# dedis/kyber

Measured on AMD Instinct MI355X. Metric: scalar-muls/s + pairings/s per node; MSM sec at 2^20 points, higher is better.
Workload: dtype int32 limbs (radix 2^25.5), int64 accumulate; 1 GPU; Ed25519 batched fixed-base + var-base scalar-mul, 2^20 scalars per GPU (BASELINE.json configs[1]); elements_per_gpu=1048576

## Files before the change

kyber_amd/csrc/ed25519.hip:

```cpp
#ifndef KYB_TU_WAVES
#define KYB_TU_WAVES 2
#endif
#include "context.h"
#include "ed25519_dev.cuh"
#include "ed25519_launch.h"
#include "msm.cuh"
#include "ed25519_h2c.cuh"
#include <stdlib.h>
#include <string.h>

#include <algorithm>
#include <atomic>
#include <chrono>
#include <thread>
#include <vector>

namespace kyb {


template <int G = 2>
__global__ void ed25519_build_base_table_kernel(int32_t* __restrict__ tab, const uint32_t* __restrict__ point,
                                                uint32_t* __restrict__ ok, int rows = ED_TAB_POS * ED_TAB_ENT) {
    const int t = blockIdx.x * blockDim.x + threadIdx.x;
    if (t >= rows) return;
// ... 102 lines not shown
        ge_p3 h;
        ge_p3_0(h);
        ge_precomp t;
        ge_p1p1 r;
        EdCombDigits<1> digits(e);
#pragma unroll 1
        for (int i = 0; i < 64; i++) {
            select_precomp_uniform(t, tab, i, digits.next(i));
            ge_madd(r, h, t);
            ge_p1p1_to_p3(h, r);
        }
        if (proj) {
            store_proj(proj, idx, h);
            continue;
        }
        uint32_t w[8];
        ge_p3_towords(w, h);
        store_words8(out + idx * 8, w);
    }
}


template <bool GTAB, bool UNI = false>
__global__ __launch_bounds__(128, 3) void ed25519_mul_kernel(
    size_t n, const uint32_t* __restrict__ scalars, const uint32_t* __restrict__ points,
    size_t points_stride, uint32_t* __restrict__ out, uint8_t* __restrict__ status,
    uint32_t flags, int32_t* __restrict__ proj, int4* __restrict__ gtab) {
    const size_t idx = (size_t)blockIdx.x * blockDim.x + threadIdx.x;
    if (idx >= n) return;
    const bool full = !UNI && (flags & KYB_F_VARTIME) != 0;
    uint32_t pw[8], a[8];
    load_words8(pw, points + idx * points_stride);
    load_words8(a, scalars + idx * 8);
    ge_p3 A;
    const bool ok = ge_p3_fromwords(A, pw);
    int8_t e[65];
    recode16(e, a, full);
    ge_p3 h;
    const int vt_top = full ? wave_top_digit(a) : 63;
    if constexpr (GTAB) {
        TabGlobal tab{gtab + idx * 80};
        ge_scalarmult_w4<UNI, true>(h, e, A, full, tab, vt_top);
    } else {
        TabScratch tab;
        ge_scalarmult_w4<UNI, true>(h, e, A, full, tab, vt_top);
    }
    if (proj) {
        store_proj(proj, idx, h);
        if (status) status[idx] = ok ? KYB_ST_OK : KYB_ST_BAD_POINT;
        return;
    }
    uint32_t w[8];
    ge_p3_towords(w, h);
    if (!ok) {
#pragma unroll
        for (int i = 0; i < 8; i++) w[i] = 0;
    }
    store_words8(out + idx * 8, w);
    if (status) status[idx] = ok ? KYB_ST_OK : KYB_ST_BAD_POINT;
}

int ed25519_build_tables(DeviceCtx* ctx) {
    KYB_HIP_CHECK(hipMalloc(&ctx->ed_base_tab, ED_TAB_WORDS * sizeof(int32_t)));
    hipLaunchKernelGGL(ed25519_build_base_table_kernel<2>, dim3((ED_TAB_POS * ED_TAB_ENT + 63) / 64), dim3(64), 0,
                       nullptr, ctx->ed_base_tab, (const uint32_t*)nullptr, (uint32_t*)nullptr, ED_TAB_POS * ED_TAB_ENT);
    KYB_HIP_CHECK(hipGetLastError());
    const auto t0 = std::chrono::steady_clock::now();
    KYB_HIP_CHECK(hipMalloc(&ctx->ed_wide_tab, ED_WIDE_WORDS * sizeof(int32_t)));
    hipLaunchKernelGGL(ed25519_build_base_table_kernel<ED_COMB_G>, dim3((EdWide::ROWS + 63) / 64), dim3(64), 0, nullptr,
                       ctx->ed_wide_tab, (const uint32_t*)nullptr, (uint32_t*)nullptr, EdWide::ROWS);
    KYB_HIP_CHECK(hipGetLastError());
    KYB_HIP_CHECK(hipStreamSynchronize(nullptr));
    ctx->ed_wide_build_us = std::chrono::duration_cast<std::chrono::microseconds>(std::chrono::steady_clock::now() - t0).count();
    return KYB_OK;
}
void ed25519_free_tables(DeviceCtx* ctx) {
    if (ctx->ed_base_tab) hipFree(ctx->ed_base_tab);
// ... 588 lines not shown
```

kyber_amd/csrc/ed25519_dev.cuh:

```cuda
#pragma once
#include "ge25519.cuh"

#if !defined(__HIPCC__)
#include <type_traits>
struct int4 { int32_t x, y, z, w; };
struct uint4 { uint32_t x, y, z, w; };
inline int4 make_int4(int32_t x, int32_t y, int32_t z, int32_t w) { return int4{x, y, z, w}; }
inline uint4 make_uint4(uint32_t x, uint32_t y, uint32_t z, uint32_t w) { return uint4{x, y, z, w}; }
#define KYB_DEV_CONST static
#else
#define KYB_DEV_CONST __device__
#endif

namespace kyb {

constexpr int ED_TAB_POS = 33;
constexpr int ED_TAB_ENT = 136;
constexpr int ED_TAB_STRIDE = 32;
constexpr int ED_TAB_WORDS = ED_TAB_POS * ED_TAB_ENT * ED_TAB_STRIDE;

template <int G>
struct EdComb {
    static constexpr int POS = (65 + G - 1) / G;
    static constexpr int POS_CT = (64 + G - 1) / G;
// ... 43 lines not shown
        ge_p1p1_to_p3(acc, r);
    }
    fe zi, x, y, ypx, ymx, xy2d, z;
    fe_invert(zi, acc.Z);
    fe_mul(x, acc.X, zi);
    fe_mul(y, acc.Y, zi);
    fe_add(ypx, y, x);
    fe_sub(ymx, y, x);
    fe_mul(xy2d, x, y);
    fe_mul(xy2d, xy2d, fe_d2());
    fe_1(z);
    fe_mul(ypx, ypx, z);
    fe_mul(ymx, ymx, z);
#pragma unroll
    for (int l = 0; l < 10; l++) {
        o[l] = ypx.v[l];
        o[10 + l] = ymx.v[l];
        o[20 + l] = xy2d.v[l];
    }
    o[30] = o[31] = 0;
}

constexpr int ENC_CHUNK = 16;

KYB_DEV void store_proj(int32_t* __restrict__ proj, size_t idx, const ge_p3& h) {
    int32_t* o = proj + idx * 30;
#pragma unroll
    for (int l = 0; l < 10; l++) {
        o[l] = h.X.v[l];
        o[10 + l] = h.Y.v[l];
        o[20 + l] = h.Z.v[l];
    }
}
KYB_DEV void load_fe(fe& f, const int32_t* __restrict__ p) {
#pragma unroll
    for (int l = 0; l < 10; l++) f.v[l] = p[l];
}
struct EncPreScratch {
    fe pre[ENC_CHUNK];
    KYB_DEV void put(int j, const fe& f) { pre[j] = f; }
    KYB_DEV void get(fe& f, int j) const { f = pre[j]; }
};
template <int LANES>
struct EncPreLds {
    int32_t* col;
    static constexpr int WORDS = ENC_CHUNK * 10 * LANES;
    KYB_DEV void put(int j, const fe& f) {
#pragma unroll
        for (int l = 0; l < 10; l++) col[(j * 10 + l) * LANES] = f.v[l];
    }
    KYB_DEV void get(fe& f, int j) const {
#pragma unroll
        for (int l = 0; l < 10; l++) f.v[l] = col[(j * 10 + l) * LANES];
        KYB_FE_MAG_SET(f, 1.01);
    }
};
#if defined(__HIPCC__)
template <int GROUP = 1>
KYB_DEV size_t ed_encode_first() {
    return (size_t)blockIdx.x * blockDim.x * (ENC_CHUNK / GROUP) + threadIdx.x;
}
#endif
template <int GROUP = 1, class Pre, class Emit>
KYB_DEV void ed_encode_chunk(size_t n, const int32_t* __restrict__ proj, size_t first, size_t stride, Pre& pre, Emit emit) {
    static_assert(GROUP >= 1 && ENC_CHUNK % GROUP == 0, "whole records per lane");
    int cnt = 0;
// ... 69 lines not shown
    }
}

template <int G>
struct EdCombDigits {
    static_assert(G >= 1 && G <= 7, "a position's digits are read from one 32-bit word");
    static constexpr int PACKED = 63 / G;
    static constexpr int TAIL = EdComb<G>::POS - PACKED;
    uint32_t pk[8];
    int tail[TAIL];
    KYB_DEV explicit EdCombDigits(const int8_t e[65]) {
        ed_pack_digits(pk, e);
#pragma unroll
        for (int t = 0; t < TAIL; t++) {
            int d = 0;
#pragma unroll
            for (int i = G - 1; i >= 0; i--)
                if (G * (PACKED + t) + i <= 64) d = 16 * d + (int)e[G * (PACKED + t) + i];
            tail[t] = d;
        }
    }
    KYB_DEV int next(int k) {
        int d = (int)(pk[0] & ((1u << (4 * G)) - 1u)) - EdComb<G>::ENT;
#pragma unroll
        for (int j = 0; j < 7; j++) pk[j] = (pk[j] >> (4 * G)) | (pk[j + 1] << (32 - 4 * G));
        pk[7] >>= 4 * G;
#pragma unroll
        for (int t = 0; t < TAIL; t++)
            if (k == PACKED + t) d = tail[t];
        return d;
    }
};

struct TabScratch {
    ge_cached tab[8];
    KYB_DEV void put(int j, const ge_cached& c) { tab[j] = c; }
    KYB_DEV void get(ge_cached& c, int j) const { c = tab[j]; }
};
struct TabGlobal {
    int4* base;
    KYB_DEV void put(int j, const ge_cached& c) {
        int4* q = base + j * 10;
        const fe* f[4] = {&c.YpX, &c.YmX, &c.Z, &c.T2d};
        int32_t w[40];
#pragma unroll
        for (int k = 0; k < 4; k++)
#pragma unroll
            for (int l = 0; l < 10; l++) w[10 * k + l] = f[k]->v[l];
#pragma unroll
        for (int i = 0; i < 10; i++) q[i] = make_int4(w[4 * i], w[4 * i + 1], w[4 * i + 2], w[4 * i + 3]);
    }
    KYB_DEV void get(ge_cached& c, int j) const {
        const int4* q = base + j * 10;
        int32_t w[40];
#pragma unroll
        for (int i = 0; i < 10; i++) {
            const int4 x = q[i];
            w[4 * i] = x.x;
            w[4 * i + 1] = x.y;
            w[4 * i + 2] = x.z;
            w[4 * i + 3] = x.w;
        }
        fe* f[4] = {&c.YpX, &c.YmX, &c.Z, &c.T2d};
#pragma unroll
        for (int k = 0; k < 4; k++)
#pragma unroll
            for (int l = 0; l < 10; l++) f[k]->v[l] = w[10 * k + l];
    }
    KYB_DEV void get_signed(ge_cached& c, int b) const;
};
KYB_DEV_CONST __attribute__((aligned(16))) const int32_t ED_CACHED_IDENTITY[40] = {1, 0, 0, 0, 0, 0, 0, 0, 0, 0,
                                                                               1, 0, 0, 0, 0, 0, 0, 0, 0, 0,
                                                                               1};
KYB_DEV void TabGlobal::get_signed(ge_cached& c, int b) const {
    const bool neg = b < 0;
    const int babs = neg ? -b : b;
#if defined(__HIPCC__)
    typedef int32_t i32x2 __attribute__((ext_vector_type(2)));
    typedef int32_t i32x4 __attribute__((ext_vector_type(4)));
    using gint = const __attribute__((address_space(1))) int32_t;
    using gint2 = const __attribute__((address_space(1))) i32x2;
    using gint4 = const __attribute__((address_space(1))) i32x4;
#else
    struct i32x2 { int32_t x, y; };
    struct i32x4 { int32_t x, y, z, w; };
    using gint = const int32_t;
    using gint2 = const i32x2;
    using gint4 = const i32x4;
#endif
    gint* e = babs ? (gint*)(base + (babs - 1) * 10) : (gint*)ED_CACHED_IDENTITY;
    gint2* p = (gint2*)(e + (neg ? 10 : 0));
    gint2* m = (gint2*)(e + (neg ? 0 : 10));
    gint4* q = (gint4*)(e + 20);
#pragma unroll
    for (int i = 0; i < 5; i++) {
        const i32x2 x = p[i], y = m[i];
        c.YpX.v[2 * i] = x.x;
        c.YpX.v[2 * i + 1] = x.y;
        c.YmX.v[2 * i] = y.x;
        c.YmX.v[2 * i + 1] = y.y;
    }
    int32_t w[20];
#pragma unroll
    for (int i = 0; i < 5; i++) {
        const i32x4 x = q[i];
        w[4 * i] = x.x;
        w[4 * i + 1] = x.y;
        w[4 * i + 2] = x.z;
        w[4 * i + 3] = x.w;
    }
    const int32_t s = -(int32_t)neg;
#pragma unroll
    for (int l = 0; l < 10; l++) {
        c.Z.v[l] = w[l];
        c.T2d.v[l] = (w[10 + l] ^ s) - s;
    }
}
template <bool UNI = false, class Tab>
KYB_DEV void select_cached(ge_cached& c, const Tab& tab, int b) {
    const bool neg = b < 0;
    const int babs = neg ? -b : b;
    if constexpr (UNI) {
        ge_cached_0(c);
#pragma unroll 1
        for (int m = 1; m <= 8; m++) {
            ge_cached x;
            tab.get(x, m - 1);
            const int32_t keep = -(int32_t)(babs == m);
#pragma unroll
            for (int l = 0; l < 10; l++) {
                c.YpX.v[l] ^= (c.YpX.v[l] ^ x.YpX.v[l]) & keep;
                c.YmX.v[l] ^= (c.YmX.v[l] ^ x.YmX.v[l]) & keep;
                c.Z.v[l] ^= (c.Z.v[l] ^ x.Z.v[l]) & keep;
                c.T2d.v[l] ^= (c.T2d.v[l] ^ x.T2d.v[l]) & keep;
            }
        }
    } else if constexpr (std::is_same_v<Tab, TabGlobal>) {
        tab.get_signed(c, b);
        return;
    } else {
        tab.get(c, babs ? babs - 1 : 0);
        if (babs == 0) ge_cached_0(c);
    }
    ge_cached_cneg(c, neg);
}

KYB_DEV int wave_top_digit(const uint32_t a[8]) {
    int bits = 0;
#pragma unroll
    for (int i = 0; i < 8; i++)
        if (a[i]) bits = 32 * i + 32 - __builtin_clz(a[i]);
    int t = (bits + 3) >> 2;
    if (t > 64) t = 64;
#if defined(__HIP_DEVICE_COMPILE__)
#pragma unroll
    for (int off = 32; off >= 1; off >>= 1) {
        const int o = __shfl_xor(t, off, 64);
        t = o > t ? o : t;
    }
    t = __builtin_amdgcn_readfirstlane(t);
#endif
    return t;
}

template <bool AFFINE = false, class Tab>
KYB_DEV void ge_window_table(Tab& tab, const ge_p3& A) {
    ge_p1p1 t;
    ge_p3 u;
    ge_cached c;
    ge_p3_to_cached(c, A);
    tab.put(0, c);
    if constexpr (AFFINE) {
        const ge_precomp a{c.YpX, c.YmX, c.T2d};
        u = A;
#pragma unroll 1
        for (int i = 0; i < 7; i++) {
            ge_madd(t, u, a);
            ge_p1p1_to_p3(u, t);
            ge_p3_to_cached(c, u);
            tab.put(i + 1, c);
        }
    } else {
#pragma unroll 1
        for (int i = 0; i < 7; i++) {
            ge_add(t, A, c);
            ge_p1p1_to_p3(u, t);
            ge_p3_to_cached(c, u);
            tab.put(i + 1, c);
        }
    }
}

template <bool UNI = false, bool AFFINE = false, class Tab>
KYB_DEV void ge_scalarmult_w4(ge_p3& h, const int8_t e[65], const ge_p3& A, bool full, Tab& tab, int vt_top) {
    ge_p1p1 t;
    ge_p3 u;
    ge_p2 r;
    ge_cached c;
    ge_window_table<AFFINE>(tab, A);
    ge_p3_0(u);
    int top = 63;
    if (full) top = vt_top;
    select_cached<UNI>(c, tab, e[top]);
    ge_add(t, u, c);
    uint32_t pk[8];
    ed_pack_digits(pk, e);
    auto shl4 = [&pk]() {
#pragma unroll
        for (int j = 7; j > 0; j--) pk[j] = (pk[j] << 4) | (pk[j - 1] >> 28);
        pk[0] <<= 4;
    };
#pragma unroll 1
    for (int i = top; i < 64; i++) shl4();
#pragma unroll 1
    for (int i = top - 1; i >= 0; i--) {
        const int d = (int)(pk[7] >> 28) - 8;
        shl4();
        ge_p1p1_to_p2(r, t);
        ge_dbl(t, r.X, r.Y, r.Z);
        ge_p1p1_to_p2(r, t);
        ge_dbl(t, r.X, r.Y, r.Z);
        ge_p1p1_to_p2(r, t);
        ge_dbl(t, r.X, r.Y, r.Z);
        ge_p1p1_to_p2(r, t);
        ge_dbl(t, r.X, r.Y, r.Z);
#if defined(__HIP_DEVICE_COMPILE__)
        if (!UNI && full && __ballot(d != 0) == 0) continue;
#endif
        ge_p1p1_to_p3(u, t);
        select_cached<UNI>(c, tab, d);
        ge_add(t, u, c);
// ... 6 lines not shown
```

kyber_amd/csrc/fe25519.cuh:

```cuda
#pragma once
#include "hd.h"

namespace kyb {

struct fe {
    int32_t v[10];
#if defined(KYB_FE_AUDIT)
    double mag = 2.0;
#endif
};

#if defined(KYB_FE_AUDIT)
inline double& fe_audit_max() {
    static double m = 0;
    return m;
}
inline double& fe_audit_max19() {
    static double m = 0;
    return m;
}
inline void fe_audit_note(double pf, double pg, double scale) {
    const double x = pf * pg * scale;
    if (x > fe_audit_max()) fe_audit_max() = x;
    if (pg > fe_audit_max19()) fe_audit_max19() = pg;
}
#define KYB_FE_MAG_SET(h, x) ((h).mag = (x))
#define KYB_FE_MAG(f) ((f).mag)
#define KYB_FE_NOTE(pf, pg, scale) fe_audit_note(pf, pg, scale)
#else
#define KYB_FE_MAG_SET(h, x) ((void)0)
#define KYB_FE_MAG(f) 0.0
#define KYB_FE_NOTE(pf, pg, scale) ((void)0)
#endif

#if defined(__HIPCC__)
#define KYB_DEV __device__ __forceinline__
#else
#define KYB_DEV inline
// ... 157 lines not shown
}
KYB_DEV void fe_sq_sel(fe& h, const fe& f, bool dbl) {
    KYB_FE_NOTE(KYB_FE_MAG(f), KYB_FE_MAG(f), 2.0);
    fe g = f;
    int32_t f2[10], f19[10], f38[10];
#pragma unroll
    for (int i = 0; i < 10; i++) {
        f2[i] = 2 * g.v[i];
        f19[i] = 19 * g.v[i];
        f38[i] = (int32_t)(2u * (uint32_t)f19[i]);
    }
    int64_t t[10];
#pragma unroll
    for (int k = 0; k < 10; k++) {
        int64_t acc = 0;
#pragma unroll
        for (int i = 0; i < 10; i++) {
            const int j = (k - i + 10) % 10;
            if (i > j) continue;
            const bool wrap = (i + j) >= 10;
            const bool both_odd = (i & 1) && (j & 1);
            const int32_t a = i == j ? g.v[i] : f2[i];
            const int32_t b = wrap ? (both_odd ? f38[j] : f19[j]) : (both_odd ? f2[j] : g.v[j]);
            acc += (int64_t)a * (int64_t)b;
        }
        t[k] = (dbl ? (acc + acc) : acc) + fe_bias(k);
    }
    fe_carry_store(h, t);
    KYB_FE_MAG_SET(h, 1.01);
}
KYB_DEV void fe_sq(fe& h, const fe& f) { fe_sq_t<false>(h, f); }
KYB_DEV void fe_sq2(fe& h, const fe& f) { fe_sq_t<true>(h, f); }

KYB_DEV void fe_sqn(fe& h, const fe& f, int n) {
    fe_sq(h, f);
#pragma unroll 1
    for (int i = 1; i < n; i++) fe_sq(h, h);
}

KYB_DEV void fe_pow_2_250_1(fe& out, fe& z11, const fe& z) {
    fe z2, z9, t, a5, a10, a20, a50, a100;
    fe_sq(z2, z);
    fe_sqn(t, z2, 2);
    fe_mul(z9, t, z);
    fe_mul(z11, z9, z2);
    fe_sq(t, z11);
    fe_mul(a5, t, z9);
    fe_sqn(t, a5, 5);
    fe_mul(a10, t, a5);
    fe_sqn(t, a10, 10);
    fe_mul(a20, t, a10);
    fe_sqn(t, a20, 20);
    fe_mul(t, t, a20);
    fe_sqn(t, t, 10);
    fe_mul(a50, t, a10);
    fe_sqn(t, a50, 50);
    fe_mul(a100, t, a50);
    fe_sqn(t, a100, 100);
    fe_mul(t, t, a100);
    fe_sqn(t, t, 50);
    fe_mul(out, t, a50);
}
KYB_DEV void fe_invert(fe& out, const fe& z) {
    fe t, z11;
    fe_pow_2_250_1(t, z11, z);
    fe_sqn(t, t, 5);
    fe_mul(out, t, z11);
}
KYB_DEV void fe_pow22523(fe& out, const fe& z) {
    fe t, z11;
    fe_pow_2_250_1(t, z11, z);
    fe_sqn(t, t, 2);
    fe_mul(out, t, z);
}

KYB_DEV void fe_towords(uint32_t w[8], const fe& f) {
    int32_t h[10];
#pragma unroll
    for (int i = 0; i < 10; i++) h[i] = f.v[i];
    int32_t q = (19 * h[9] + (1 << 24)) >> 25;
#pragma unroll
    for (int i = 0; i < 10; i++) q = (h[i] + q) >> ((i & 1) ? 25 : 26);
    h[0] += 19 * q;
#pragma unroll
    for (int i = 0; i < 9; i++) {
        const int w_ = (i & 1) ? 25 : 26;
        int32_t c = h[i] >> w_;
        h[i + 1] += c;
        h[i] -= c << w_;
    }
    h[9] &= (1 << 25) - 1;
    uint32_t u[10];
#pragma unroll
    for (int i = 0; i < 10; i++) u[i] = (uint32_t)h[i];
    w[0] = u[0] | (u[1] << 26);
    w[1] = (u[1] >> 6) | (u[2] << 19);
    w[2] = (u[2] >> 13) | (u[3] << 13);
    w[3] = (u[3] >> 19) | (u[4] << 6);
    w[4] = u[5] | (u[6] << 25);
    w[5] = (u[6] >> 7) | (u[7] << 19);
    w[6] = (u[7] >> 13) | (u[8] << 12);
    w[7] = (u[8] >> 20) | (u[9] << 6);
}
KYB_DEV void fe_fromwords(fe& h, const uint32_t w[8]) {
    h.v[0] = (int32_t)(w[0] & 0x3ffffff);
    h.v[1] = (int32_t)(((w[0] >> 26) | (w[1] << 6)) & 0x1ffffff);
    h.v[2] = (int32_t)(((w[1] >> 19) | (w[2] << 13)) & 0x3ffffff);
    h.v[3] = (int32_t)(((w[2] >> 13) | (w[3] << 19)) & 0x1ffffff);
    h.v[4] = (int32_t)((w[3] >> 6) & 0x3ffffff);
    h.v[5] = (int32_t)(w[4] & 0x1ffffff);
    h.v[6] = (int32_t)(((w[4] >> 25) | (w[5] << 7)) & 0x3ffffff);
    h.v[7] = (int32_t)(((w[5] >> 19) | (w[6] << 13)) & 0x1ffffff);
    h.v[8] = (int32_t)(((w[6] >> 12) | (w[7] << 20)) & 0x3ffffff);
    h.v[9] = (int32_t)((w[7] >> 6) & 0x1ffffff);
    KYB_FE_MAG_SET(h, 2.0);
}
KYB_DEV bool fe_isnegative(const fe& f) {
    uint32_t w[8];
    fe_towords(w, f);
    return w[0] & 1;
}
KYB_DEV bool fe_isnonzero(const fe& f) {
// ... 10 lines not shown
```

kyber_amd/csrc/ge25519.cuh:

```cuda
#pragma once
#include "fe25519.cuh"

namespace kyb {

struct ge_p2 { fe X, Y, Z; };
struct ge_p3 { fe X, Y, Z, T; };
struct ge_p1p1 { fe X, Y, Z, T; };
struct ge_cached { fe YpX, YmX, Z, T2d; };
struct ge_precomp { fe ypx, ymx, xy2d; };

#include "ed25519_consts.inc"

KYB_DEV void ge_p3_0(ge_p3& h) {
    fe_0(h.X);
    fe_1(h.Y);
    fe_1(h.Z);
    fe_0(h.T);
}
KYB_DEV void ge_cached_0(ge_cached& c) {
    fe_1(c.YpX);
    fe_1(c.YmX);
    fe_1(c.Z);
    fe_0(c.T2d);
}
KYB_DEV void ge_p1p1_to_p2(ge_p2& r, const ge_p1p1& p) {
    fe_mul(r.X, p.X, p.T);
    fe_mul(r.Y, p.Y, p.Z);
    fe_mul(r.Z, p.Z, p.T);
}
KYB_DEV void ge_p1p1_to_p3(ge_p3& r, const ge_p1p1& p) {
    fe_mul(r.X, p.X, p.T);
    fe_mul(r.Y, p.Y, p.Z);
    fe_mul(r.Z, p.Z, p.T);
    fe_mul(r.T, p.X, p.Y);
}
KYB_DEV void ge_p3_to_cached(ge_cached& r, const ge_p3& p) {
    fe_add(r.YpX, p.Y, p.X);
    fe_sub(r.YmX, p.Y, p.X);
    r.Z = p.Z;
    fe_mul(r.T2d, p.T, fe_d2());
}
KYB_DEV void ge_dbl(ge_p1p1& r, const fe& X, const fe& Y, const fe& Z) {
    fe t0;
    fe_sq(r.X, X);
    fe_sq(r.Z, Y);
    fe_sq2(r.T, Z);
    fe_add(r.Y, X, Y);
    fe_sq(t0, r.Y);
    fe_add(r.Y, r.Z, r.X);
    fe_sub(r.Z, r.Z, r.X);
    fe_sub(r.X, t0, r.Y);
    fe_sub(r.T, r.T, r.Z);
}
KYB_DEV void ge_add(ge_p1p1& r, const ge_p3& p, const ge_cached& q) {
    fe t0;
    fe_add(r.X, p.Y, p.X);
    fe_sub(r.Y, p.Y, p.X);
    fe_mul(r.Z, r.X, q.YpX);
    fe_mul(r.Y, r.Y, q.YmX);
    fe_mul(r.T, q.T2d, p.T);
    fe_mul(r.X, p.Z, q.Z);
    fe_add(t0, r.X, r.X);
    fe_sub(r.X, r.Z, r.Y);
    fe_add(r.Y, r.Z, r.Y);
    fe_add(r.Z, t0, r.T);
    fe_sub(r.T, t0, r.T);
}
KYB_DEV void ge_madd(ge_p1p1& r, const ge_p3& p, const ge_precomp& q) {
    fe t0;
    fe_add(r.X, p.Y, p.X);
    fe_sub(r.Y, p.Y, p.X);
    fe_mul(r.Z, r.X, q.ypx);
    fe_mul(r.Y, r.Y, q.ymx);
    fe_mul(r.T, q.xy2d, p.T);
    fe_add(t0, p.Z, p.Z);
    fe_sub(r.X, r.Z, r.Y);
    fe_add(r.Y, r.Z, r.Y);
    fe_add(r.Z, t0, r.T);
    fe_sub(r.T, t0, r.T);
}
KYB_DEV void ge_cached_cneg(ge_cached& c, bool neg) {
    fe_cswap(c.YpX, c.YmX, neg);
    fe nt;
    fe_neg(nt, c.T2d);
    fe_cmov(c.T2d, nt, neg);
}
KYB_DEV void ge_precomp_cneg(ge_precomp& c, bool neg) {
    fe_cswap(c.ypx, c.ymx, neg);
    fe nt;
    fe_neg(nt, c.xy2d);
    fe_cmov(c.xy2d, nt, neg);
}

KYB_DEV void ge_encode_with_zinv(uint32_t w[8], const fe& X, const fe& Y, const fe& zinv) {
    fe x, y;
    fe_mul(x, X, zinv);
    fe_mul(y, Y, zinv);
    fe_towords(w, y);
    w[7] ^= (uint32_t)fe_isnegative(x) << 31;
}
KYB_DEV void ge_p3_towords(uint32_t w[8], const ge_p3& p) {
    fe zi;
    fe_invert(zi, p.Z);
    ge_encode_with_zinv(w, p.X, p.Y, zi);
}
KYB_DEV bool ge_p3_fromwords(ge_p3& p, const uint32_t w[8]) {
    fe u, v, v3, vxx, check;
    fe_fromwords(p.Y, w);
    fe_1(p.Z);
    fe_sq(u, p.Y);
    fe_mul(v, u, fe_d());
    fe_sub(u, u, p.Z);
    fe_add(v, v, p.Z);
    fe_sq(v3, v);
    fe_mul(v3, v3, v);
    fe_sq(p.X, v3);
    fe_mul(p.X, p.X, v);
    fe_mul(p.X, p.X, u);
    fe_pow22523(p.X, p.X);
    fe_mul(p.X, p.X, v3);
    fe_mul(p.X, p.X, u);
    fe_sq(vxx, p.X);
    fe_mul(vxx, vxx, v);
    fe_sub(check, vxx, u);
    bool ok = true;
    if (fe_isnonzero(check)) {
        fe_add(check, vxx, u);
        ok = !fe_isnonzero(check);
        fe xs;
        fe_mul(xs, p.X, fe_sqrtm1());
        p.X = xs;
    }
    const bool sign = (w[7] >> 31) != 0;
    fe nx;
    fe_neg(nx, p.X);
    fe_cmov(p.X, nx, fe_isnegative(p.X) != sign);
    fe_mul(p.T, p.X, p.Y);
    return ok;
}

KYB_DEV void recode16(int8_t e[65], const uint32_t a[8], bool full256) {
    int carry = 0;
#pragma unroll
    for (int i = 0; i < 64; i++) {
        int d = (int)((a[i >> 3] >> ((i & 7) * 4)) & 15) + carry;
        if (i < 63) {
            carry = (d + 8) >> 4;
            d -= carry << 4;
        }
        e[i] = (int8_t)d;
    }
    int top = e[63];
    int c2 = 0;
    if (full256) {
        c2 = (top + 8) >> 4;
        top -= c2 << 4;
    } else if (top > 8) {
        top = 0;
    }
    e[63] = (int8_t)top;
    e[64] = (int8_t)c2;
}

KYB_DEV bool ed_effective_scalar(uint32_t (&k)[8]) {
    uint32_t c = 0, t7 = 0;
#pragma unroll
    for (int j = 0; j < 8; j++) {
// ... 21 lines not shown
```

kyber_amd/csrc/gen_consts.py:

```python
#!/usr/bin/env python3
import os

HERE = os.path.dirname(os.path.abspath(__file__))


def limbs_25_5(x):
    out, off = [], 0
    for i in range(10):
        w = 25 if i & 1 else 26
        out.append((x >> off) & ((1 << w) - 1))
        off += w
    assert off == 255 and x >> 255 == 0
    return out


def ed25519():
    p = 2**255 - 19
    d = (-121665 * pow(121666, p - 2, p)) % p
    sqrtm1 = pow(2, (p - 1) // 4, p)
    by = 4 * pow(5, p - 2, p) % p
    u, v = (by * by - 1) % p, (d * by * by + 1) % p
    bx = (u * pow(v, 3, p) * pow(u * pow(v, 7, p) % p, (p - 5) // 8, p)) % p
    if (v * bx * bx - u) % p:
        bx = bx * sqrtm1 % p
    assert (v * bx * bx - u) % p == 0
    if bx & 1:
        bx = p - bx
    a = (-486664) % p
    c1 = pow(a, (p + 3) // 8, p)
    if c1 * c1 % p != a:
        c1 = c1 * sqrtm1 % p
    assert c1 * c1 % p == a
    if c1 & 1:
        c1 = p - c1
    c2 = pow(2, (p + 3) // 8, p)
    consts = dict(d=d, d2=2 * d % p, sqrtm1=sqrtm1, bx=bx, by=by, bt=bx * by % p, elligator_c1=c1, elligator_c2=c2)
    lines = ["// generated by gen_consts.py -- do not edit"]
    for name, val in consts.items():
        ls = ", ".join(str(v) for v in limbs_25_5(val))
        lines.append(f"KYB_DEV fe fe_{name}() {{ return fe{{{{{ls}}}}}; }}")
    open(os.path.join(HERE, "ed25519_consts.inc"), "w").write("\n".join(lines) + "\n")



def _limbs(x, n, w):
    assert x >> (n * w) == 0
    return [(x >> (w * i)) & ((1 << w) - 1) for i in range(n)]


def _words(x, nw):
    assert x >> (32 * nw) == 0
    return [(x >> (32 * i)) & 0xFFFFFFFF for i in range(nw)]


def _arr(vals):
    return "{" + ", ".join("0x%xu" % v for v in vals) + "}"


class MontField:
    def __init__(self, p, n, w, nwords):
        self.p, self.n, self.w, self.nwords = p, n, w, nwords
        self.R = 1 << (n * w)
        assert self.R > 4 * p and 32 * nwords <= n * w

    def mont(self, x):
        return _words(x % self.p * self.R % self.p, self.nwords)

    def mont2(self, c):
        return "{" + _arr(self.mont(c[0])) + ", " + _arr(self.mont(c[1])) + "}"

    def emit(self, name, extra=""):
        p, n, w = self.p, self.n, self.w
        ninv = (-pow(p, -1, 1 << w)) % (1 << w)
        nw = self.nwords
        L = [f"struct {name} {{",
# ... 234 lines not shown
```

Measured before the change: 181.3 million scalar-muls/s.

## Switch variable-base Ed25519 scalar-mul to 9-limb radix-2^29 field arithmetic

Adds a new 9-limb radix-2^29 field element type (fe29) with 64-bit accumulating schoolbook multiply/square and a lazy signed-limb carry chain using a 2^261 fold constant. The geometry routines and window tables are templated over field type, and the variable-base mul kernel now runs the w4 scalar-mult entirely in fe29, with a smaller 9-int4 global table entry. The aim is fewer limb products per field multiply (81 vs 100) and less table traffic, in exchange for 64-bit accumulation, costlier carry handling and conversions on input and output.

```diff
diff --git a/kyber_amd/csrc/ed25519.hip b/kyber_amd/csrc/ed25519.hip
--- a/kyber_amd/csrc/ed25519.hip
+++ b/kyber_amd/csrc/ed25519.hip
@@ -158,17 +158,17 @@
     uint32_t pw[8], a[8];
     load_words8(pw, points + idx * points_stride);
     load_words8(a, scalars + idx * 8);
-    ge_p3 A;
+    ge29_p3 A;
     const bool ok = ge_p3_fromwords(A, pw);
     int8_t e[65];
     recode16(e, a, full);
-    ge_p3 h;
+    ge29_p3 h;
     const int vt_top = full ? wave_top_digit(a) : 63;
     if constexpr (GTAB) {
-        TabGlobal tab{gtab + idx * 80};
+        TabGlobal_t<fe29> tab{gtab + idx * 80};
         ge_scalarmult_w4<UNI, true>(h, e, A, full, tab, vt_top);
     } else {
-        TabScratch tab;
+        TabScratch_t<fe29> tab;
         ge_scalarmult_w4<UNI, true>(h, e, A, full, tab, vt_top);
     }
     if (proj) {
diff --git a/kyber_amd/csrc/ed25519_consts29.inc b/kyber_amd/csrc/ed25519_consts29.inc
--- /dev/null
+++ b/kyber_amd/csrc/ed25519_consts29.inc
@@ -0,0 +1,3 @@
+KYB_DEV fe29 fe29_d() { return fe29{{324630691, 257584720, 276179677, 1350274, 512327687, 3980220, 432943901, 499478015, 5374828}}; }
+KYB_DEV fe29 fe29_d2() { return fe29{{112390489, 515169441, 15488442, 2700549, 487784462, 7960441, 329016890, 462085119, 2361049}}; }
+KYB_DEV fe29 fe29_sqrtm1() { return fe29{{168730800, 124836154, 200875569, 103812442, 494564084, 5021437, 472689972, 269088827, 2851620}}; }
diff --git a/kyber_amd/csrc/ed25519_dev.cuh b/kyber_amd/csrc/ed25519_dev.cuh
--- a/kyber_amd/csrc/ed25519_dev.cuh
+++ b/kyber_amd/csrc/ed25519_dev.cuh
@@ -99,6 +99,13 @@
         o[20 + l] = h.Z.v[l];
     }
 }
+KYB_DEV void store_proj(int32_t* __restrict__ proj, size_t idx, const ge29_p3& h) {
+    ge_p3 t;
+    fe29_to_fe(t.X, h.X);
+    fe29_to_fe(t.Y, h.Y);
+    fe29_to_fe(t.Z, h.Z);
+    store_proj(proj, idx, t);
+}
 KYB_DEV void load_fe(fe& f, const int32_t* __restrict__ p) {
 #pragma unroll
     for (int l = 0; l < 10; l++) f.v[l] = p[l];
@@ -234,12 +241,19 @@
     }
 };
 
-struct TabScratch {
-    ge_cached tab[8];
-    KYB_DEV void put(int j, const ge_cached& c) { tab[j] = c; }
-    KYB_DEV void get(ge_cached& c, int j) const { c = tab[j]; }
-};
-struct TabGlobal {
+template <class F = fe>
+struct TabScratch_t {
+    typedef typename ge_t<F>::cached cached;
+    cached tab[8];
+    KYB_DEV void put(int j, const cached& c) { tab[j] = c; }
+    KYB_DEV void get(cached& c, int j) const { c = tab[j]; }
+};
+using TabScratch = TabScratch_t<>;
+template <class F = fe>
+struct TabGlobal_t;
+using TabGlobal = TabGlobal_t<>;
+template <>
+struct TabGlobal_t<fe> {
     int4* base;
     KYB_DEV void put(int j, const ge_cached& c) {
         int4* q = base + j * 10;
@@ -274,7 +288,7 @@
 KYB_DEV_CONST __attribute__((aligned(16))) const int32_t ED_CACHED_IDENTITY[40] = {1, 0, 0, 0, 0, 0, 0, 0, 0, 0,
                                                                                1, 0, 0, 0, 0, 0, 0, 0, 0, 0,
                                                                                1};
-KYB_DEV void TabGlobal::get_signed(ge_cached& c, int b) const {
+KYB_DEV void TabGlobal_t<fe>::get_signed(ge_cached& c, int b) const {
     const bool neg = b < 0;
     const int babs = neg ? -b : b;
 #if defined(__HIPCC__)
@@ -318,26 +332,118 @@
         c.T2d.v[l] = (w[10 + l] ^ s) - s;
     }
 }
-template <bool UNI = false, class Tab>
-KYB_DEV void select_cached(ge_cached& c, const Tab& tab, int b) {
+template <>
+struct TabGlobal_t<fe29> {
+    int4* base;
+    static constexpr int word(int field, int l) { return field < 2 ? (l < 8 ? 8 * field + l : 16 + field) : 18 + 9 * (field - 2) + l; }
+    KYB_DEV void put(int j, const ge29_cached& c) {
+        int4* q = base + j * 9;
+        const fe29* f[4] = {&c.YpX, &c.YmX, &c.Z, &c.T2d};
+        int32_t w[36];
+#pragma unroll
+        for (int k = 0; k < 4; k++)
+#pragma unroll
+            for (int l = 0; l < 9; l++) w[word(k, l)] = f[k]->v[l];
+#pragma unroll
+        for (int i = 0; i < 9; i++) q[i] = make_int4(w[4 * i], w[4 * i + 1], w[4 * i + 2], w[4 * i + 3]);
+    }
+    KYB_DEV void get(ge29_cached& c, int j) const {
+        const int4* q = base + j * 9;
+        int32_t w[36];
+#pragma unroll
+        for (int i = 0; i < 9; i++) {
+            const int4 x = q[i];
+            w[4 * i] = x.x;
+            w[4 * i + 1] = x.y;
+            w[4 * i + 2] = x.z;
+            w[4 * i + 3] = x.w;
+        }
+        fe29* f[4] = {&c.YpX, &c.YmX, &c.Z, &c.T2d};
+#pragma unroll
+        for (int k = 0; k < 4; k++)
+#pragma unroll
+            for (int l = 0; l < 9; l++) f[k]->v[l] = w[word(k, l)];
+        KYB_FE_MAG_SET(c.YpX, 3.001);
+        KYB_FE_MAG_SET(c.YmX, 3.001);
+        KYB_FE_MAG_SET(c.Z, 1.001);
+        KYB_FE_MAG_SET(c.T2d, 1.001);
+    }
+    KYB_DEV void get_signed(ge29_cached& c, int b) const;
+};
+KYB_DEV_CONST __attribute__((aligned(16))) const int32_t ED_CACHED_IDENTITY29[36] = {1, 0, 0, 0, 0, 0, 0, 0,
+                                                                                 1, 0, 0, 0, 0, 0, 0, 0,
+                                                                                 0, 0, 1};
+KYB_DEV void TabGlobal_t<fe29>::get_signed(ge29_cached& c, int b) const {
+    const bool neg = b < 0;
+    const int babs = neg ? -b : b;
+#if defined(__HIPCC__)
+    typedef int32_t i32x4 __attribute__((ext_vector_type(4)));
+    using gint = const __attribute__((address_space(1))) int32_t;
+    using gint4 = const __attribute__((address_space(1))) i32x4;
+#else
+    struct i32x4 { int32_t x, y, z, w; };
+    using gint = const int32_t;
+    using gint4 = const i32x4;
+#endif
+    gint* e = babs ? (gint*)(base + (babs - 1) * 9) : (gint*)ED_CACHED_IDENTITY29;
+    gint4* p = (gint4*)(e + (neg ? 8 : 0));
+    gint4* m = (gint4*)(e + (neg ? 0 : 8));
+    gint4* q = (gint4*)(e + 16);
+#pragma unroll
+    for (int i = 0; i < 2; i++) {
+        const i32x4 x = p[i], y = m[i];
+        c.YpX.v[4 * i] = x.x;
+        c.YpX.v[4 * i + 1] = x.y;
+        c.YpX.v[4 * i + 2] = x.z;
+        c.YpX.v[4 * i + 3] = x.w;
+        c.YmX.v[4 * i] = y.x;
+        c.YmX.v[4 * i + 1] = y.y;
+        c.YmX.v[4 * i + 2] = y.z;
+        c.YmX.v[4 * i + 3] = y.w;
+    }
+    int32_t w[20];
+#pragma unroll
+    for (int i = 0; i < 5; i++) {
+        const i32x4 x = q[i];
+        w[4 * i] = x.x;
+        w[4 * i + 1] = x.y;
+        w[4 * i + 2] = x.z;
+        w[4 * i + 3] = x.w;
+    }
+    c.YpX.v[8] = neg ? w[1] : w[0];
+    c.YmX.v[8] = neg ? w[0] : w[1];
+    const int32_t s = -(int32_t)neg;
+#pragma unroll
+    for (int l = 0; l < 9; l++) {
+        c.Z.v[l] = w[2 + l];
+        c.T2d.v[l] = (w[11 + l] ^ s) - s;
+    }
+    KYB_FE_MAG_SET(c.YpX, 3.001);
+    KYB_FE_MAG_SET(c.YmX, 3.001);
+    KYB_FE_MAG_SET(c.Z, 1.001);
+    KYB_FE_MAG_SET(c.T2d, 1.001);
+}
+template <bool UNI = false, class C, class Tab>
+KYB_DEV void select_cached(C& c, const Tab& tab, int b) {
+    typedef decltype(c.Z) F;
     const bool neg = b < 0;
     const int babs = neg ? -b : b;
     if constexpr (UNI) {
         ge_cached_0(c);
 #pragma unroll 1
         for (int m = 1; m <= 8; m++) {
-            ge_cached x;
+            C x;
             tab.get(x, m - 1);
             const int32_t keep = -(int32_t)(babs == m);
 #pragma unroll
-            for (int l = 0; l < 10; l++) {
+            for (int l = 0; l < F::N; l++) {
                 c.YpX.v[l] ^= (c.YpX.v[l] ^ x.YpX.v[l]) & keep;
                 c.YmX.v[l] ^= (c.YmX.v[l] ^ x.YmX.v[l]) & keep;
                 c.Z.v[l] ^= (c.Z.v[l] ^ x.Z.v[l]) & keep;
                 c.T2d.v[l] ^= (c.T2d.v[l] ^ x.T2d.v[l]) & keep;
             }
         }
-    } else if constexpr (std::is_same_v<Tab, TabGlobal>) {
+    } else if constexpr (std::is_same_v<Tab, TabGlobal_t<F>>) {
         tab.get_signed(c, b);
         return;
     } else {
@@ -365,15 +471,16 @@
     return t;
 }
 
-template <bool AFFINE = false, class Tab>
-KYB_DEV void ge_window_table(Tab& tab, const ge_p3& A) {
-    ge_p1p1 t;
-    ge_p3 u;
-    ge_cached c;
+template <bool AFFINE = false, class P3, class Tab>
+KYB_DEV void ge_window_table(Tab& tab, const P3& A) {
+    typedef ge_t<decltype(A.X)> G;
+    typename G::p1p1 t;
+    P3 u;
+    typename G::cached c;
     ge_p3_to_cached(c, A);
     tab.put(0, c);
     if constexpr (AFFINE) {
-        const ge_precomp a{c.YpX, c.YmX, c.T2d};
+        const typename G::precomp a{c.YpX, c.YmX, c.T2d};
         u = A;
 #pragma unroll 1
         for (int i = 0; i < 7; i++) {
@@ -393,12 +500,13 @@
     }
 }
 
-template <bool UNI = false, bool AFFINE = false, class Tab>
-KYB_DEV void ge_scalarmult_w4(ge_p3& h, const int8_t e[65], const ge_p3& A, bool full, Tab& tab, int vt_top) {
-    ge_p1p1 t;
-    ge_p3 u;
-    ge_p2 r;
-    ge_cached c;
+template <bool UNI = false, bool AFFINE = false, class P3, class Tab>
+KYB_DEV void ge_scalarmult_w4(P3& h, const int8_t e[65], const P3& A, bool full, Tab& tab, int vt_top) {
+    typedef ge_t<decltype(A.X)> G;
+    typename G::p1p1 t;
+    P3 u;
+    typename G::p2 r;
+    typename G::cached c;
     ge_window_table<AFFINE>(tab, A);
     ge_p3_0(u);
     int top = 63;
diff --git a/kyber_amd/csrc/fe25519.cuh b/kyber_amd/csrc/fe25519.cuh
--- a/kyber_amd/csrc/fe25519.cuh
+++ b/kyber_amd/csrc/fe25519.cuh
@@ -4,6 +4,7 @@
 namespace kyb {
 
 struct fe {
+    static constexpr int N = 10;
     int32_t v[10];
 #if defined(KYB_FE_AUDIT)
     double mag = 2.0;
@@ -227,14 +228,16 @@
 KYB_DEV void fe_sq(fe& h, const fe& f) { fe_sq_t<false>(h, f); }
 KYB_DEV void fe_sq2(fe& h, const fe& f) { fe_sq_t<true>(h, f); }
 
-KYB_DEV void fe_sqn(fe& h, const fe& f, int n) {
+template <class F>
+KYB_DEV void fe_sqn(F& h, const F& f, int n) {
     fe_sq(h, f);
 #pragma unroll 1
     for (int i = 1; i < n; i++) fe_sq(h, h);
 }
 
-KYB_DEV void fe_pow_2_250_1(fe& out, fe& z11, const fe& z) {
-    fe z2, z9, t, a5, a10, a20, a50, a100;
+template <class F>
+KYB_DEV void fe_pow_2_250_1(F& out, F& z11, const F& z) {
+    F z2, z9, t, a5, a10, a20, a50, a100;
     fe_sq(z2, z);
     fe_sqn(t, z2, 2);
     fe_mul(z9, t, z);
@@ -256,14 +259,16 @@
     fe_sqn(t, t, 50);
     fe_mul(out, t, a50);
 }
-KYB_DEV void fe_invert(fe& out, const fe& z) {
-    fe t, z11;
+template <class F>
+KYB_DEV void fe_invert(F& out, const F& z) {
+    F t, z11;
     fe_pow_2_250_1(t, z11, z);
     fe_sqn(t, t, 5);
     fe_mul(out, t, z11);
 }
-KYB_DEV void fe_pow22523(fe& out, const fe& z) {
-    fe t, z11;
+template <class F>
+KYB_DEV void fe_pow22523(F& out, const F& z) {
+    F t, z11;
     fe_pow_2_250_1(t, z11, z);
     fe_sqn(t, t, 2);
     fe_mul(out, t, z);
@@ -282,7 +287,7 @@
         const int w_ = (i & 1) ? 25 : 26;
         int32_t c = h[i] >> w_;
         h[i + 1] += c;
-        h[i] -= c << w_;
+        h[i] -= c * (1 << w_);
     }
     h[9] &= (1 << 25) - 1;
     uint32_t u[10];
diff --git a/kyber_amd/csrc/fe29.cuh b/kyber_amd/csrc/fe29.cuh
--- /dev/null
+++ b/kyber_amd/csrc/fe29.cuh
@@ -0,0 +1,255 @@
+#pragma once
+#include "fe25519.cuh"
+
+namespace kyb {
+
+struct fe29 {
+    static constexpr int N = 9;
+    int32_t v[9];
+#if defined(KYB_FE_AUDIT)
+    double mag = 2.0;
+#endif
+};
+
+constexpr double FE29_MUL_LIMIT = 14.0;
+constexpr double FE29_SQ_LIMIT = 3.99;
+constexpr int32_t FE29_MASK = (1 << 29) - 1;
+constexpr int32_t FE29_FOLD = 1216;
+
+#if defined(KYB_FE_AUDIT)
+inline double& fe29_audit_max() {
+    static double m = 0;
+    return m;
+}
+inline double& fe29_audit_max_sq() {
+    static double m = 0;
+    return m;
+}
+inline void fe29_audit_note(double pf, double pg, double scale, bool sq) {
+    const double x = pf * pg * scale;
+    if (x > fe29_audit_max()) fe29_audit_max() = x;
+    if (sq && pf > fe29_audit_max_sq()) fe29_audit_max_sq() = pf;
+}
+#define KYB_FE29_NOTE(pf, pg, scale, sq) fe29_audit_note(pf, pg, scale, sq)
+#else
+#define KYB_FE29_NOTE(pf, pg, scale, sq) ((void)0)
+#endif
+
+KYB_DEV void fe_0(fe29& h) {
+#pragma unroll
+    for (int i = 0; i < 9; i++) h.v[i] = 0;
+    KYB_FE_MAG_SET(h, 0.0);
+}
+KYB_DEV void fe_1(fe29& h) {
+    fe_0(h);
+    h.v[0] = 1;
+    KYB_FE_MAG_SET(h, 1.0 / (1 << 28));
+}
+KYB_DEV void fe_add(fe29& h, const fe29& f, const fe29& g) {
+    const double m_ = KYB_FE_MAG(f) + KYB_FE_MAG(g);
+#pragma unroll
+    for (int i = 0; i < 9; i++) h.v[i] = f.v[i] + g.v[i];
+    KYB_FE_MAG_SET(h, m_);
+    (void)m_;
+}
+KYB_DEV void fe_sub(fe29& h, const fe29& f, const fe29& g) {
+    const double m_ = KYB_FE_MAG(f) + KYB_FE_MAG(g);
+#pragma unroll
+    for (int i = 0; i < 9; i++) h.v[i] = f.v[i] - g.v[i];
+    KYB_FE_MAG_SET(h, m_);
+    (void)m_;
+}
+KYB_DEV void fe_neg(fe29& h, const fe29& f) {
+    const double m_ = KYB_FE_MAG(f);
+#pragma unroll
+    for (int i = 0; i < 9; i++) h.v[i] = -f.v[i];
+    KYB_FE_MAG_SET(h, m_);
+    (void)m_;
+}
+KYB_DEV void fe_cmov(fe29& f, const fe29& g, bool b) {
+#pragma unroll
+    for (int i = 0; i < 9; i++) f.v[i] = b ? g.v[i] : f.v[i];
+    KYB_FE_MAG_SET(f, KYB_FE_MAG(f) > KYB_FE_MAG(g) ? KYB_FE_MAG(f) : KYB_FE_MAG(g));
+}
+KYB_DEV void fe_cswap(fe29& f, fe29& g, bool b) {
+#pragma unroll
+    for (int i = 0; i < 9; i++) {
+        int32_t x = f.v[i], y = g.v[i];
+        f.v[i] = b ? y : x;
+        g.v[i] = b ? x : y;
+    }
+    const double m_ = KYB_FE_MAG(f) > KYB_FE_MAG(g) ? KYB_FE_MAG(f) : KYB_FE_MAG(g);
+    KYB_FE_MAG_SET(f, m_);
+    KYB_FE_MAG_SET(g, m_);
+    (void)m_;
+}
+
+KYB_DEV int32_t fe29_fold() {
+    int32_t k = FE29_FOLD;
+#if defined(__HIP_DEVICE_COMPILE__)
+    asm("" : "+s"(k));
+#endif
+    return k;
+}
+
+KYB_DEV constexpr int64_t fe29_bias(int k) {
+    return (k & 1) ? 0 : ((int64_t)1 << 28) + (k < 8 ? ((int64_t)1 << 57) : 0);
+}
+
+template <class HiF>
+KYB_DEV int32_t fe29_high(int32_t lo[8], HiF hi) {
+    int64_t c = 0;
+#pragma unroll
+    for (int k = 9; k < 17; k++) {
+        const int64_t T = hi(k, c);
+        lo[k - 9] = (int32_t)((uint32_t)T & (uint32_t)FE29_MASK);
+        c = T >> 29;
+    }
+    return (int32_t)c;
+}
+template <class ColF>
+KYB_DEV void fe29_chain_store(fe29& h, ColF col) {
+    int32_t r[9];
+    const int64_t T0 = col(0, fe29_bias(0));
+    int64_t c = T0 >> 29;
+    const uint32_t b0 = (uint32_t)T0 & (uint32_t)FE29_MASK;
+#pragma unroll
+    for (int k = 1; k < 9; k++) {
+        const int64_t T = (k & 1) ? col(k, c) : col(k, fe29_bias(k)) + c;
+        c = T >> 29;
+        r[k] = (int32_t)((uint32_t)T & (uint32_t)FE29_MASK) - (1 << 28);
+    }
+    const int64_t t0 = (int64_t)b0 + c * FE29_FOLD;
+    c = t0 >> 29;
+    r[0] = (int32_t)((uint32_t)t0 & (uint32_t)FE29_MASK) - (1 << 28);
+    r[1] += (int32_t)c;
+#pragma unroll
+    for (int i = 0; i < 9; i++) h.v[i] = r[i];
+}
+
+KYB_DEV void fe_mul(fe29& h, const fe29& f, const fe29& g) {
+    KYB_FE29_NOTE(KYB_FE_MAG(f), KYB_FE_MAG(g), 1.0, false);
+    const int32_t fold = fe29_fold();
+    int32_t lo[9];
+    lo[8] = fe29_high(lo, [&](int k, int64_t acc) {
+#pragma unroll
+        for (int i = k - 8; i < 9; i++) {
+            acc += (int64_t)f.v[i] * (int64_t)g.v[k - i];
+            KYB_PIN64(acc);
+        }
+        return acc;
+    });
+    fe29_chain_store(h, [&](int k, int64_t acc) {
+#pragma unroll
+        for (int i = 0; i <= k; i++) {
+            acc += (int64_t)f.v[i] * (int64_t)g.v[k - i];
+            KYB_PIN64(acc);
+        }
+        acc += (int64_t)lo[k] * (int64_t)fold;
+        KYB_PIN64(acc);
+        return acc;
+    });
+    KYB_FE_MAG_SET(h, 1.001);
+}
+
+template <bool DBL>
+KYB_DEV void fe29_sq_t(fe29& h, const fe29& f) {
+    KYB_FE29_NOTE(KYB_FE_MAG(f), KYB_FE_MAG(f), DBL ? 2.0 : 1.0, true);
+    const int32_t fold = fe29_fold();
+    int32_t f2[9];
+#pragma unroll
+    for (int i = 0; i < 9; i++) f2[i] = 2 * f.v[i];
+    auto products = [&](int k, int64_t acc) {
+#pragma unroll
+        for (int i = (k > 8 ? k - 8 : 0); 2 * i <= k; i++) {
+            const int j = k - i;
+            const int32_t a = (i == j && !DBL) ? f.v[i] : f2[i];
+            const int32_t b = (i == j || !DBL) ? f.v[j] : f2[j];
+            acc += (int64_t)a * (int64_t)b;
+            KYB_PIN64(acc);
+        }
+        return acc;
+    };
+    int32_t lo[9];
+    lo[8] = fe29_high(lo, products);
+    fe29_chain_store(h, [&](int k, int64_t acc) {
+        acc = products(k, acc);
+        acc += (int64_t)lo[k] * (int64_t)fold;
+        KYB_PIN64(acc);
+        return acc;
+    });
+    KYB_FE_MAG_SET(h, 1.001);
+}
+KYB_DEV void fe_sq(fe29& h, const fe29& f) { fe29_sq_t<false>(h, f); }
+KYB_DEV void fe_sq2(fe29& h, const fe29& f) { fe29_sq_t<true>(h, f); }
+
+KYB_DEV void fe_fromwords(fe29& h, const uint32_t w[8]) {
+#pragma unroll
+    for (int i = 0; i < 9; i++) {
+        const int o = 29 * i, j = o / 32, s = o % 32;
+        uint32_t x = w[j] >> s;
+        if (s + 29 > 32 && j + 1 < 8) x |= w[j + 1] << (32 - s);
+        h.v[i] = (int32_t)(x & (uint32_t)(i < 8 ? FE29_MASK : (1 << 23) - 1));
+    }
+    KYB_FE_MAG_SET(h, 2.0);
+}
+KYB_DEV void fe_towords(uint32_t w[8], const fe29& f) {
+    int32_t h[9];
+#pragma unroll
+    for (int i = 0; i < 9; i++) h[i] = f.v[i];
+#pragma unroll
+    for (int pass = 0; pass < 2; pass++) {
+#pragma unroll
+        for (int i = 0; i < 8; i++) {
+            h[i + 1] += h[i] >> 29;
+            h[i] &= FE29_MASK;
+        }
+        h[0] += 19 * (h[8] >> 23);
+        h[8] &= (1 << 23) - 1;
+    }
+    int32_t q = (h[0] + 19) >> 29;
+#pragma unroll
+    for (int i = 1; i < 8; i++) q = (h[i] + q) >> 29;
+    q = (h[8] + q) >> 23;
+    h[0] += 19 * q;
+#pragma unroll
+    for (int i = 0; i < 8; i++) {
+        h[i + 1] += h[i] >> 29;
+        h[i] &= FE29_MASK;
+    }
+    h[8] &= (1 << 23) - 1;
+#pragma unroll
+    for (int j = 0; j < 8; j++) w[j] = 0;
+#pragma unroll
+    for (int i = 0; i < 9; i++) {
+        const int o = 29 * i, j = o / 32, s = o % 32;
+        w[j] |= (uint32_t)h[i] << s;
+        if (s + 29 > 32 && j + 1 < 8) w[j + 1] |= (uint32_t)h[i] >> (32 - s);
+    }
+}
+KYB_DEV bool fe_isnegative(const fe29& f) {
+    uint32_t w[8];
+    fe_towords(w, f);
+    return w[0] & 1;
+}
+KYB_DEV bool fe_isnonzero(const fe29& f) {
+    uint32_t w[8];
+    fe_towords(w, f);
+    uint32_t r = 0;
+#pragma unroll
+    for (int i = 0; i < 8; i++) r |= w[i];
+    return r != 0;
+}
+
+KYB_DEV void fe29_to_fe(fe& h, const fe29& f) {
+    uint32_t w[8];
+    fe_towords(w, f);
+    fe_fromwords(h, w);
+}
+KYB_DEV void fe29_from_fe(fe29& h, const fe& f) {
+    uint32_t w[8];
+    fe_towords(w, f);
+    fe_fromwords(h, w);
+}
+
+}
diff --git a/kyber_amd/csrc/ge25519.cuh b/kyber_amd/csrc/ge25519.cuh
--- a/kyber_amd/csrc/ge25519.cuh
+++ b/kyber_amd/csrc/ge25519.cuh
@@ -1,5 +1,6 @@
 #pragma once
 #include "fe25519.cuh"
+#include "fe29.cuh"
 
 namespace kyb {
 
@@ -8,40 +9,70 @@
 struct ge_p1p1 { fe X, Y, Z, T; };
 struct ge_cached { fe YpX, YmX, Z, T2d; };
 struct ge_precomp { fe ypx, ymx, xy2d; };
+struct ge29_p2 { fe29 X, Y, Z; };
+struct ge29_p3 { fe29 X, Y, Z, T; };
+struct ge29_p1p1 { fe29 X, Y, Z, T; };
+struct ge29_cached { fe29 YpX, YmX, Z, T2d; };
+struct ge29_precomp { fe29 ypx, ymx, xy2d; };
+template <class F> struct ge_t;
+template <> struct ge_t<fe> {
+    typedef ge_p2 p2; typedef ge_p3 p3; typedef ge_p1p1 p1p1; typedef ge_cached cached; typedef ge_precomp precomp;
+};
+template <> struct ge_t<fe29> {
+    typedef ge29_p2 p2; typedef ge29_p3 p3; typedef ge29_p1p1 p1p1; typedef ge29_cached cached; typedef ge29_precomp precomp;
+};
 
 #include "ed25519_consts.inc"
-
-KYB_DEV void ge_p3_0(ge_p3& h) {
+#include "ed25519_consts29.inc"
+template <class F> struct fe_k;
+template <> struct fe_k<fe> {
+    static KYB_DEV fe d() { return fe_d(); }
+    static KYB_DEV fe d2() { return fe_d2(); }
+    static KYB_DEV fe sqrtm1() { return fe_sqrtm1(); }
+};
+template <> struct fe_k<fe29> {
+    static KYB_DEV fe29 d() { return fe29_d(); }
+    static KYB_DEV fe29 d2() { return fe29_d2(); }
+    static KYB_DEV fe29 sqrtm1() { return fe29_sqrtm1(); }
+};
+
+template <class P3>
+KYB_DEV void ge_p3_0(P3& h) {
     fe_0(h.X);
     fe_1(h.Y);
     fe_1(h.Z);
     fe_0(h.T);
 }
-KYB_DEV void ge_cached_0(ge_cached& c) {
+template <class C>
+KYB_DEV void ge_cached_0(C& c) {
     fe_1(c.YpX);
     fe_1(c.YmX);
     fe_1(c.Z);
     fe_0(c.T2d);
 }
-KYB_DEV void ge_p1p1_to_p2(ge_p2& r, const ge_p1p1& p) {
+template <class P2, class P1>
+KYB_DEV void ge_p1p1_to_p2(P2& r, const P1& p) {
     fe_mul(r.X, p.X, p.T);
     fe_mul(r.Y, p.Y, p.Z);
     fe_mul(r.Z, p.Z, p.T);
 }
-KYB_DEV void ge_p1p1_to_p3(ge_p3& r, const ge_p1p1& p) {
+template <class P3, class P1>
+KYB_DEV void ge_p1p1_to_p3(P3& r, const P1& p) {
     fe_mul(r.X, p.X, p.T);
     fe_mul(r.Y, p.Y, p.Z);
     fe_mul(r.Z, p.Z, p.T);
     fe_mul(r.T, p.X, p.Y);
 }
-KYB_DEV void ge_p3_to_cached(ge_cached& r, const ge_p3& p) {
+template <class C, class P3>
+KYB_DEV void ge_p3_to_cached(C& r, const P3& p) {
     fe_add(r.YpX, p.Y, p.X);
     fe_sub(r.YmX, p.Y, p.X);
     r.Z = p.Z;
-    fe_mul(r.T2d, p.T, fe_d2());
-}
-KYB_DEV void ge_dbl(ge_p1p1& r, const fe& X, const fe& Y, const fe& Z) {
-    fe t0;
+    fe_mul(r.T2d, p.T, fe_k<decltype(p.T)>::d2());
+}
+template <class P1, class F>
+KYB_DEV void ge_dbl(P1& r, const F& X, const F& Y, const F& Z) {
+    F t0;
     fe_sq(r.X, X);
     fe_sq(r.Z, Y);
     fe_sq2(r.T, Z);
@@ -52,8 +83,9 @@
     fe_sub(r.X, t0, r.Y);
     fe_sub(r.T, r.T, r.Z);
 }
-KYB_DEV void ge_add(ge_p1p1& r, const ge_p3& p, const ge_cached& q) {
-    fe t0;
+template <class P1, class P3, class C>
+KYB_DEV void ge_add(P1& r, const P3& p, const C& q) {
+    decltype(p.X) t0;
     fe_add(r.X, p.Y, p.X);
     fe_sub(r.Y, p.Y, p.X);
     fe_mul(r.Z, r.X, q.YpX);
@@ -66,8 +98,9 @@
     fe_add(r.Z, t0, r.T);
     fe_sub(r.T, t0, r.T);
 }
-KYB_DEV void ge_madd(ge_p1p1& r, const ge_p3& p, const ge_precomp& q) {
-    fe t0;
+template <class P1, class P3, class C>
+KYB_DEV void ge_madd(P1& r, const P3& p, const C& q) {
+    decltype(p.X) t0;
     fe_add(r.X, p.Y, p.X);
     fe_sub(r.Y, p.Y, p.X);
     fe_mul(r.Z, r.X, q.ypx);
@@ -79,9 +112,10 @@
     fe_add(r.Z, t0, r.T);
     fe_sub(r.T, t0, r.T);
 }
-KYB_DEV void ge_cached_cneg(ge_cached& c, bool neg) {
+template <class C>
+KYB_DEV void ge_cached_cneg(C& c, bool neg) {
     fe_cswap(c.YpX, c.YmX, neg);
-    fe nt;
+    decltype(c.T2d) nt;
     fe_neg(nt, c.T2d);
     fe_cmov(c.T2d, nt, neg);
 }
@@ -92,24 +126,28 @@
     fe_cmov(c.xy2d, nt, neg);
 }
 
-KYB_DEV void ge_encode_with_zinv(uint32_t w[8], const fe& X, const fe& Y, const fe& zinv) {
-    fe x, y;
+template <class F>
+KYB_DEV void ge_encode_with_zinv(uint32_t w[8], const F& X, const F& Y, const F& zinv) {
+    F x, y;
     fe_mul(x, X, zinv);
     fe_mul(y, Y, zinv);
     fe_towords(w, y);
     w[7] ^= (uint32_t)fe_isnegative(x) << 31;
 }
-KYB_DEV void ge_p3_towords(uint32_t w[8], const ge_p3& p) {
-    fe zi;
+template <class P3>
+KYB_DEV void ge_p3_towords(uint32_t w[8], const P3& p) {
+    decltype(p.Z) zi;
     fe_invert(zi, p.Z);
     ge_encode_with_zinv(w, p.X, p.Y, zi);
 }
-KYB_DEV bool ge_p3_fromwords(ge_p3& p, const uint32_t w[8]) {
-    fe u, v, v3, vxx, check;
+template <class P3>
+KYB_DEV bool ge_p3_fromwords(P3& p, const uint32_t w[8]) {
+    typedef decltype(p.X) F;
+    F u, v, v3, vxx, check;
     fe_fromwords(p.Y, w);
     fe_1(p.Z);
     fe_sq(u, p.Y);
-    fe_mul(v, u, fe_d());
+    fe_mul(v, u, fe_k<F>::d());
     fe_sub(u, u, p.Z);
     fe_add(v, v, p.Z);
     fe_sq(v3, v);
@@ -127,12 +165,12 @@
     if (fe_isnonzero(check)) {
         fe_add(check, vxx, u);
         ok = !fe_isnonzero(check);
-        fe xs;
-        fe_mul(xs, p.X, fe_sqrtm1());
+        F xs;
+        fe_mul(xs, p.X, fe_k<F>::sqrtm1());
         p.X = xs;
     }
     const bool sign = (w[7] >> 31) != 0;
-    fe nx;
+    F nx;
     fe_neg(nx, p.X);
     fe_cmov(p.X, nx, fe_isnegative(p.X) != sign);
     fe_mul(p.T, p.X, p.Y);
diff --git a/kyber_amd/csrc/gen_consts.py b/kyber_amd/csrc/gen_consts.py
--- a/kyber_amd/csrc/gen_consts.py
+++ b/kyber_amd/csrc/gen_consts.py
@@ -40,7 +40,11 @@
         ls = ", ".join(str(v) for v in limbs_25_5(val))
         lines.append(f"KYB_DEV fe fe_{name}() {{ return fe{{{{{ls}}}}}; }}")
     open(os.path.join(HERE, "ed25519_consts.inc"), "w").write("\n".join(lines) + "\n")
-
+    lines = ["// generated by gen_consts.py -- do not edit"]
+    for name in ("d", "d2", "sqrtm1"):
+        ls = ", ".join(str(v) for v in _limbs(consts[name], 9, 29))
+        lines.append(f"KYB_DEV fe29 fe29_{name}() {{ return fe29{{{{{ls}}}}}; }}")
+    open(os.path.join(HERE, "ed25519_consts29.inc"), "w").write("\n".join(lines) + "\n")
 
 
 def _limbs(x, n, w):
```

After: 190.4 million scalar-muls/s, median of 6. 5.1% higher.
